# lupalab/posterior-matching

Measured on AMD Instinct MI355X. Metric: training images/sec, PM-VAE MNIST bs=256 per GPU (ELBO / PM matching-LL in `aux`), higher is better.
Workload: dtype bf16x3; 1 GPU; configs/pm_vae_mnist.py: conv PM-VAE 28x28x1, latent 32, TriL posterior, AR-GMM partial posterior, Bernoulli decoder; full train step (fwd+loss+bwd+Adam); per_gpu_batch=256, global_batch=256, parallelism=dp1, launch=launch_plan_2streams, params=2101969, rccl_ranks=1

## Files before the change

include/pmhip.h:

```cpp
#ifndef PMHIP_H
#define PMHIP_H

#ifdef __cplusplus
extern "C" {
#endif

#define PM_OK 0
#define PM_EINVAL (-1)
#define PM_ELAUNCH (-2)

#define PM_ACT_NONE 0
#define PM_ACT_LEAKY 1
#define PM_ACT_RELU 2
#define PM_ACT_GELU 3
#define PM_AUX_AFTER_RES 16

typedef void* pm_stream_t;

typedef struct pm_gather_desc {
    int B;
    int IH, IW, C;
    int OH, OW, N;
    int KH, KW;
    int a, cs, off, d;
    int wts, wcs, wns;
    int groups;
    long long in_gs, w_gs, out_gs, bias_gs;
    int in_act, out_act, aux_act;
    float slope;
    int off_x, kws;
} pm_gather_desc;

int pm_gather_gemm(pm_stream_t stream, const pm_gather_desc* d, const float* in, const float* w,
                   const float* bias, const float* aux, const float* res, float* out);

int pm_gather_wgrad(pm_stream_t stream, const pm_gather_desc* d, const float* gathered,
                    const float* dense, float* dw, float* db);

int pm_gather_gemm_bf16(pm_stream_t stream, const pm_gather_desc* d, const float* in, const void* wsplit,
                        const float* bias, const float* aux, const float* res, float* out);
int pm_gather_gemm_bf16_dual(pm_stream_t stream, const pm_gather_desc* d, const float* in, const void* wsplit,
                             const float* bias, const float* aux, const float* res, float* out, float* out2, int act2);
int pm_gemm_splitk_floats(const pm_gather_desc* d, int bf16, int in_aligned16, long long* floats);
int pm_gather_gemm_sk(pm_stream_t stream, const pm_gather_desc* d, const float* in, const float* w, const float* bias,
                      const float* aux, const float* res, float* out, float* scratch, long long scratch_floats);
int pm_gather_gemm_bf16_sk(pm_stream_t stream, const pm_gather_desc* d, const float* in, const void* wsplit,
                           const float* bias, const float* aux, const float* res, float* out, float* out2, int act2,
                           float* scratch, long long scratch_floats);
int pm_gather_gemm_bf16_insum(pm_stream_t stream, const pm_gather_desc* d, const float* in, const void* wsplit,
                              const float* bias, const float* aux, const float* res, float* out, float* in_colsum);
int pm_image_conv_insum_applies(const pm_gather_desc* d);

int pm_gather_wgrad_bf16(pm_stream_t stream, const pm_gather_desc* d, const float* gathered, const float* dense,
                         float* dw, float* db);

typedef struct pm_split_job {
    long long src_off;
    long long dst_off;
    long long plane;
    int taps, C, N, npad;
    int wts, wcs, wns;
    int first_block, num_blocks;
    int kw, kws;
    int dense_k;
} pm_split_job;
int pm_split_weights(pm_stream_t stream, const float* params, void* out_bf16, const pm_split_job* jobs_dev,
                     int njobs, int total_blocks);

int pm_thin_conv(pm_stream_t stream, const pm_gather_desc* d, const float* in, const float* w, const float* bias,
                 const float* aux, const float* res, float* out);
int pm_thin_wgrad(pm_stream_t stream, const pm_gather_desc* d, const float* gathered, const float* dense, float* dw,
                  float* db, float* db_gathered);
int pm_thin_to1_bf16(pm_stream_t stream, const pm_gather_desc* d, const float* in, const float* w, const float* bias,
                     const float* aux, const float* res, float* out);
int pm_tap_shift_add(pm_stream_t stream, const pm_gather_desc* d, const float* T, int ldt, const float* bias,
                     float* out);

int pm_gather_wgrad_table(pm_stream_t stream, const pm_gather_desc* d, const float* gathered, const float* dense, float* dw,
                          float* db, const long long* table, int all_aligned16, int use_bf16);

int pm_query_gemm_plan(const pm_gather_desc* d, int in_aligned16, int* bm, int* bn, int* vec);
int pm_query_wgrad_plan(const pm_gather_desc* d, int gathered_aligned16, int dense_aligned16, int* rc, int* rn,
                        int* vec, int* dvec, int* workgroups);

int pm_mask_concat(pm_stream_t stream, const float* x, const float* b, float* out, long long R, int C, int Cb);

int pm_tril_sample_kl_fwd(pm_stream_t stream, const float* params, const float* eps, float* z, float* kl, int B, int k);
int pm_tril_sample_kl_bwd(pm_stream_t stream, const float* params, const float* eps, const float* dz,
                          const float* g_kl, float* dparams, int B, int k);
int pm_tril_sample_kl_bwd2(pm_stream_t stream, const float* params, const float* eps, const float* dz, const float* dz2,
                           const float* g_kl, float* dparams, int B, int k);
int pm_tril_logprob_fwd(pm_stream_t stream, const float* params, const float* z, float* lp, int B, int k);
int pm_tril_logprob_bwd(pm_stream_t stream, const float* params, const float* z, const float* g,
                        float* dparams, float* dz , int B, int k);

int pm_diag_gaussian_sample_kl_fwd(pm_stream_t stream, const float* params, const float* eps, float* z, float* kl, int B, int k);
int pm_diag_gaussian_sample_kl_bwd(pm_stream_t stream, const float* params, const float* eps, const float* dz,
                                   const float* g_kl, float* dparams, int B, int k);
int pm_diag_gaussian_logprob_fwd(pm_stream_t stream, const float* params, const float* z, float* lp, int B, int k);
int pm_diag_gaussian_logprob_bwd(pm_stream_t stream, const float* params, const float* z, const float* g, float* dparams,
                                 float* dz, int B, int k);

int pm_bernoulli_ll_fwd(pm_stream_t stream, const float* logits, const float* x, float* ll, int B, int D);
int pm_bernoulli_ll_bwd(pm_stream_t stream, const float* logits, const float* x, const float* g, float* dpre,
                        int B, int D, int act, float slope);
int pm_bernoulli_ll_fwd_bwd(pm_stream_t stream, const float* logits, const float* x, const float* g, float* ll, float* dpre,
                            int B, int D, int act, float slope);

int pm_normal_ll_fwd(pm_stream_t stream, const float* loc, const float* x, const float* log_scale, float* ll, int B,
                     int D, float scale_eps);
int pm_normal_ll_bwd(pm_stream_t stream, const float* loc, const float* x, const float* log_scale, const float* g,
                     float* dloc, float* d_log_scale, int B, int D, float scale_eps);
int pm_normal_ll_bwd_det(pm_stream_t stream, const float* loc, const float* x, const float* log_scale, const float* g,
                         float* dloc, float* d_log_scale, int B, int D, float scale_eps, float* scratch);

int pm_argmm_build_input(pm_stream_t stream, const float* z, const float* ctx, float* inp, int B, int k, int ctx_dim);
int pm_argmm_input_bwd(pm_stream_t stream, const float* dinp, float* dz, float* dctx, int B, int k, int ctx_dim,
                       int accumulate_dz, const float* ctx, int ctx_act, float slope);
int pm_gmm_logprob_fwd(pm_stream_t stream, const float* head, const float* z, float* mll, int B, int k, int nc);
int pm_gmm_logprob_bwd(pm_stream_t stream, const float* head, const float* z, const float* g, float* dhead,
                       float* dz, int B, int k, int nc, int accumulate_dz);

int pm_vq_select(pm_stream_t stream, const float* z, const float* emb, const float* dots, float* e2, int* idx,
                 float* quant, float* commit_grad, float* sqerr, float* counts, float* dw, int N, int D, int K,
                 float commit_coef);
int pm_vq_dw_exact_floats(int N, int D, int K, long long* floats);
int pm_vq_dw_exact(pm_stream_t stream, const float* z, const int* idx, float* dw, int N, int D, int K, float* scratch,
                   long long scratch_floats);
int pm_embed_bwd_sorted(pm_stream_t stream, const int* idx, const float* dout, float* dtable, long long rows, int F, int K,
                        float* scratch, long long scratch_floats);
int pm_vq_ema_update(pm_stream_t stream, const float* counts, const float* dw, float* cs_hidden, float* cs_avg,
                     float* dw_hidden, float* dw_avg, float* emb, int* counter, int D, int K, float decay,
                     float epsilon);
int pm_vq_lookup(pm_stream_t stream, const int* idx, const float* emb, float* quant, int N, int D, int K);
// ... 276 lines not shown
```

posterior_matching_amd/_lib.py:

```python
from __future__ import annotations

import ctypes as C
import os

_HERE = os.path.dirname(os.path.abspath(__file__))
LIB_PATH = os.environ.get("PM_LIB_PATH") or os.path.join(_HERE, "lib", "libpmhip.so")

ACT_NONE, ACT_LEAKY, ACT_RELU, ACT_GELU = 0, 1, 2, 3
AUX_AFTER_RES = 16
LEAKY_SLOPE = 0.01


class PmHipError(RuntimeError):
    pass


class GatherDesc(C.Structure):

    _fields_ = [
        ("B", C.c_int),
        ("IH", C.c_int), ("IW", C.c_int), ("C", C.c_int),
        ("OH", C.c_int), ("OW", C.c_int), ("N", C.c_int),
        ("KH", C.c_int), ("KW", C.c_int),
        ("a", C.c_int), ("cs", C.c_int), ("off", C.c_int), ("d", C.c_int),
# ... 12 lines not shown
        ("low", C.c_float), ("high", C.c_float),
        ("period_or_steps", C.c_int), ("delay_or_begin", C.c_int),
        ("matching_coef", C.c_float),
        ("grad_scale", C.c_float),
    ]


class AdamCfg(C.Structure):
    _fields_ = [
        ("b1", C.c_float), ("b2", C.c_float), ("eps", C.c_float), ("weight_decay", C.c_float),
        ("lr_init", C.c_float), ("lr_decay_rate", C.c_float), ("lr_transition_steps", C.c_float),
        ("grad_scale", C.c_float),
        ("lr_kind", C.c_int), ("lr_end", C.c_float), ("zero_grad", C.c_int),
    ]


class MaskComponent(C.Structure):

    _fields_ = [
        ("kind", C.c_int), ("p", C.c_float),
        ("y1", C.c_int), ("x1", C.c_int), ("y2", C.c_int), ("x2", C.c_int),
        ("size", C.c_int), ("min_prop", C.c_float), ("max_prop", C.c_float), ("cum_weight", C.c_float),
    ]


class VdvaeBlockIO(C.Structure):

    _fields_ = [
        ("x", C.c_void_p), ("x2", C.c_void_p), ("res", C.c_void_p), ("xpre", C.c_void_p), ("xg_out", C.c_void_p),
        ("h", C.c_void_p * 3), ("g", C.c_void_p * 3), ("out", C.c_void_p),
        ("w", C.c_void_p * 4), ("plane", C.c_longlong * 4), ("bias", C.c_void_p * 4),
        ("Cin", C.c_int), ("Cout", C.c_int), ("Ca", C.c_int), ("dense_k3", C.c_int),
    ]


class SplitJob(C.Structure):

    _fields_ = [
        ("src_off", C.c_longlong), ("dst_off", C.c_longlong), ("plane", C.c_longlong),
        ("taps", C.c_int), ("C", C.c_int), ("N", C.c_int), ("npad", C.c_int),
        ("wts", C.c_int), ("wcs", C.c_int), ("wns", C.c_int),
        ("first_block", C.c_int), ("num_blocks", C.c_int),
        ("kw", C.c_int), ("kws", C.c_int), ("dense_k", C.c_int),
    ]


class WgradPart(C.Structure):

    _fields_ = [
        ("w", C.c_void_p), ("b", C.c_void_p), ("bg", C.c_void_p),
        ("w_stride", C.c_longlong), ("b_stride", C.c_longlong), ("bg_stride", C.c_longlong),
        ("nslots", C.c_int),
    ]


class ColsumJob(C.Structure):
    _fields_ = [("x", C.c_void_p), ("part", C.c_void_p), ("part_stride", C.c_longlong), ("M", C.c_longlong),
                ("N", C.c_int), ("nslots", C.c_int)]


class ReduceJob(C.Structure):

    _fields_ = [
        ("src", C.c_void_p), ("stride", C.c_longlong), ("g_off", C.c_longlong),
        ("count", C.c_int), ("nslots", C.c_int),
    ]


_P = C.c_void_p
_I = C.c_int
_LL = C.c_longlong
_F = C.c_float

SIGNATURES = {
    "pm_gather_gemm": [_P, C.POINTER(GatherDesc), _P, _P, _P, _P, _P, _P],
    "pm_gather_wgrad": [_P, C.POINTER(GatherDesc), _P, _P, _P, _P],
    "pm_gather_gemm_bf16": [_P, C.POINTER(GatherDesc), _P, _P, _P, _P, _P, _P],
    "pm_gather_gemm_bf16_dual": [_P, C.POINTER(GatherDesc), _P, _P, _P, _P, _P, _P, _P, _I],
    "pm_gemm_splitk_floats": [C.POINTER(GatherDesc), _I, _I, C.POINTER(C.c_longlong)],
    "pm_gather_gemm_sk": [_P, C.POINTER(GatherDesc), _P, _P, _P, _P, _P, _P, _P, C.c_longlong],
    "pm_gather_gemm_bf16_sk": [_P, C.POINTER(GatherDesc), _P, _P, _P, _P, _P, _P, _P, _I, _P, C.c_longlong],
    "pm_gather_gemm_bf16_insum": [_P, C.POINTER(GatherDesc), _P, _P, _P, _P, _P, _P, _P],
    "pm_image_conv_insum_applies": [C.POINTER(GatherDesc)],
    "pm_split_weights": [_P, _P, _P, _P, _I, _I],
    "pm_gather_wgrad_bf16": [_P, C.POINTER(GatherDesc), _P, _P, _P, _P],
    "pm_gather_wgrad_table": [_P, C.POINTER(GatherDesc), _P, _P, _P, _P, _P, _I, _I],
    "pm_wgrad_part_slots": [C.POINTER(GatherDesc), _P, _P, _I, _I, _I, C.POINTER(_I)],
    "pm_gather_wgrad_part": [_P, C.POINTER(GatherDesc), _P, _P, _P, _I, _I, C.POINTER(WgradPart)],
    "pm_thin_wgrad_part_slots": [C.POINTER(GatherDesc), _P, _P, C.POINTER(_I)],
    "pm_thin_wgrad_part": [_P, C.POINTER(GatherDesc), _P, _P, C.POINTER(WgradPart)],
    "pm_colsum_part_slots": [_LL, _I, C.POINTER(_I)],
    "pm_colsum_part": [_P, _P, _LL, _I, _P, _LL, _I],
    "pm_colsum_part_multi": [_P, _P, _I],
    "pm_reduce_partials": [_P, _P, _I, _P],
    "pm_adam_step_jobs": [_P, _P, _I, _P, _P, _P, _P, _LL, _P, C.POINTER(AdamCfg)],
    "pm_thin_conv": [_P, C.POINTER(GatherDesc), _P, _P, _P, _P, _P, _P],
    "pm_thin_wgrad": [_P, C.POINTER(GatherDesc), _P, _P, _P, _P, _P],
    "pm_thin_to1_bf16": [_P, C.POINTER(GatherDesc), _P, _P, _P, _P, _P, _P],
    "pm_tap_shift_add": [_P, C.POINTER(GatherDesc), _P, _I, _P, _P],
    "pm_mask_concat": [_P, _P, _P, _P, _LL, _I, _I],
    "pm_tril_sample_kl_fwd": [_P, _P, _P, _P, _P, _I, _I],
    "pm_tril_sample_kl_bwd": [_P, _P, _P, _P, _P, _P, _I, _I],
    "pm_tril_logprob_fwd": [_P, _P, _P, _P, _I, _I],
    "pm_tril_logprob_bwd": [_P, _P, _P, _P, _P, _P, _I, _I],
    "pm_diag_gaussian_sample_kl_fwd": [_P, _P, _P, _P, _P, _I, _I],
    "pm_diag_gaussian_sample_kl_bwd": [_P, _P, _P, _P, _P, _P, _I, _I],
    "pm_diag_gaussian_logprob_fwd": [_P, _P, _P, _P, _I, _I],
    "pm_diag_gaussian_logprob_bwd": [_P, _P, _P, _P, _P, _P, _I, _I],
    "pm_bernoulli_ll_fwd": [_P, _P, _P, _P, _I, _I],
    "pm_bernoulli_ll_bwd": [_P, _P, _P, _P, _P, _I, _I, _I, _F],
    "pm_bernoulli_ll_fwd_bwd": [_P, _P, _P, _P, _P, _P, _I, _I, _I, _F],
    "pm_tril_sample_kl_bwd2": [_P, _P, _P, _P, _P, _P, _P, _I, _I],
    "pm_normal_ll_fwd": [_P, _P, _P, _P, _P, _I, _I, _F],
    "pm_normal_ll_bwd": [_P, _P, _P, _P, _P, _P, _P, _I, _I, _F],
    "pm_normal_ll_bwd_det": [_P, _P, _P, _P, _P, _P, _P, _I, _I, _F, _P],
    "pm_vq_select": [_P, _P, _P, _P, _P, _P, _P, _P, _P, _P, _P, _I, _I, _I, _F],
    "pm_vq_dw_exact": [_P, _P, _P, _P, _I, _I, _I, _P, C.c_longlong],
    "pm_embed_bwd_sorted": [_P, _P, _P, _P, C.c_longlong, _I, _I, _P, C.c_longlong],
    "pm_vq_dw_exact_floats": [_I, _I, _I, C.POINTER(C.c_longlong)],
    "pm_vq_ema_update": [_P, _P, _P, _P, _P, _P, _P, _P, _P, _I, _I, _F, _F],
    "pm_vq_lookup": [_P, _P, _P, _P, _I, _I, _I],
    "pm_vqvae_loss": [_P, _P, _P, _P, _I, _I, _I, _I, _F, _F, _P, _P],
    "pm_argmm_build_input": [_P, _P, _P, _P, _I, _I, _I],
    "pm_argmm_input_bwd": [_P, _P, _P, _P, _I, _I, _I, _I, _P, _I, _F],
    "pm_gmm_logprob_fwd": [_P, _P, _P, _P, _I, _I, _I],
    "pm_gmm_logprob_bwd": [_P, _P, _P, _P, _P, _P, _I, _I, _I, _I],
    "pm_embed_fwd": [_P, _P, _P, _P, _LL, _I, _I],
    "pm_embed_bwd": [_P, _P, _P, _P, _LL, _I, _I],
    "pm_embed_bwd_exact": [_P, _P, _P, _P, _LL, _I, _I, _P],
    "pm_concat_elu_fwd": [_P, _P, _P, _P, _P, _LL, _I, _I],
    "pm_concat_elu_bwd": [_P, _P, _P, _P, _P, _P, _P, _LL, _I, _I, _I, _P],
    "pm_gate_bwd_rows_sum": [_P, _P, _P, _P, _P, _P, _LL, _I, _I],
    "pm_concat_elu_fwd_philox": [_P, _P, _P, _P, _LL, _I, _I, _F, C.c_ulonglong, _P, _I],
    "pm_concat_elu_bwd_philox": [_P, _P, _P, _P, _P, _P, _LL, _I, _I, _I, _P, _F, C.c_ulonglong, _P, _I],
    "pm_gate_fwd": [_P, _P, _P, _P, _P, _LL, _I, _I],
    "pm_gate_fwd_ce": [_P, _P, _P, _P, _P, _P, _LL, _I, _I],
    "pm_gate_bwd": [_P, _P, _P, _P, _P, _LL, _I, _I],
    "pm_rows_sum": [_P, _P, _P, _LL, _I, _I],
    "pm_rows_sum_multi": [_P, _P, _I, _P, C.c_longlong, _I, _I],
    "pm_groups_sum": [_P, _P, _P, _LL, _I, _LL, _I],
    "pm_elu_fwd": [_P, _P, _P, _LL],
    "pm_elu_bwd": [_P, _P, _P, _P, _LL, _I],
    "pm_categorical_ll_fwd": [_P, _P, _P, _P, _P, _LL, _I, _I],
    "pm_categorical_ll_bwd": [_P, _P, _P, _P, _P, _P, _LL, _I, _I],
    "pm_neg_mean_loss": [_P, _P, _I, _F, _P, _P],
    "pm_categorical_sample": [_P, _P, _P, _P, _LL, _I, _I, _I],
    "pm_impute_blend": [_P, _P, _P, _P, _LL, _I, _LL, _I, _I, _F, _F],
    "pm_imputation_psnr": [_P, _P, _P, _P, _LL, _I, _LL, _F],
    "pm_gumbel_fill": [_P, _P, _LL, C.c_ulonglong, _P, _I],
    "pm_mlp_pair_bf16": [_P, _P, _P, _P, _P, _P, _P, _P, _P, _P, _LL, _I, _I, _I, _I, _I, _F],
    "pm_info_gain_inputs": [_P, _P, _P, _P, _P, _I, _I, _I],
    "pm_gaussian_entropy": [_P, _P, _P, _LL, _I, _I, _I],
    "pm_info_gain_finish": [_P, _P, _P, _P, _I, _I],
    "pm_sample_project_fwd": [_P, _P, _P, _I, _P, _P, _P, _P, _P, _P, _P, _LL, _I, _I, _I],
    "pm_sample_project_bwd": [_P, _P, _P, _I, _P, _P, _P, _F, _P, _P, _LL, _I, _I],
    "pm_mlp_chain_bf16": [_P, _P, _I, _P, _P, _P, _P, _LL, _I, _I, _I, _I, _F],
    "pm_repeat_rows": [_P, _P, _P, _LL, _I, _LL],
    "pm_sigmoid": [_P, _P, _P, _LL],
    "pm_bernoulli_ll_rep_fwd": [_P, _P, _P, _P, _P, _I, _I, _I, _I],
    "pm_normal_ll_rep_fwd": [_P, _P, _P, _P, _P, _P, _I, _I, _I, _I, _F],
    "pm_std_normal_logprob": [_P, _P, _P, _LL, _I],
    "pm_logmeanexp3": [_P, _P, _P, _P, _P, _I, _I, _I],
    "pm_gmm_sample_step": [_P, _P, _P, _P, _P, _LL, _I, _I, _I],
    "pm_diag_logprob_acc": [_P, _P, _I, _P, _P, _LL, _I, _I, _F],
    "pm_segment_wsum": [_P, _P, _P, _P, _I, _I, _F, _I],
    "pm_image_mask_mixture": [_P, _P, _I, _I, _I, C.POINTER(MaskComponent), _I, C.c_ulonglong, _P, _I, _P, _P,
# ... 108 lines not shown
```

posterior_matching_amd/models/networks.py:

```python
from __future__ import annotations

from typing import Any, Dict, List, Optional, Sequence, Tuple

import torch

from .. import ops
from ..ops import ACT_LEAKY, ACT_NONE, ACT_RELU, LayerGeom
from .core import Feat, Module, ParamStore


class ConvEncoder(Module):

    def __init__(self, conv_layers: Sequence[Tuple[int, int, int]], name: Optional[str] = None):
        super().__init__(name)
        self._conv_layers = [tuple(l) for l in conv_layers]

    def build(self, store: ParamStore, prefix: str, in_shape) -> Tuple[int, ...]:
        if len(in_shape) != 3:
            raise ValueError(f"ConvEncoder expects [H, W, C] inputs, got {tuple(in_shape)}")
        self.attach(store, prefix)
        h, w, c = in_shape
        self.geoms: List[LayerGeom] = []
        self._ws = []
        n = len(self._conv_layers)
        for i, (f, k, s) in enumerate(self._conv_layers):
            g = LayerGeom.conv(h, w, c, f, k, s, "VALID" if i == n - 1 else "SAME")
            store.add(f"{prefix}/conv_{i}/w", g.weight_shape, fan_in=k * k * c)
            store.add(f"{prefix}/conv_{i}/b", (f,))
            self.geoms.append(g)
            self._ws.append((store.request_split(f"{prefix}/conv_{i}/w", g, "fwd"),
                             store.request_split(f"{prefix}/conv_{i}/w", g, "dgrad")))
            h, w, c = g.OH, g.OW, f
        return (h, w, c)

    def __call__(self, x: Feat, is_training: bool = False) -> Feat:
        assert x.in_act == ACT_NONE
        B = x.t.shape[0]
        self._x = x
        self._outs = []
        h = x.t
        for i, g in enumerate(self.geoms):
            out = self.buf(f"out_{i}", (B, g.OH, g.OW, g.CO))
            ops.layer_forward(g, h, self.P(f"conv_{i}/w"), self.P(f"conv_{i}/b"), out, out_act=ACT_LEAKY,
                              wsplit=self.store.split_view(self._ws[i][0]))
            self._outs.append(out)
            h = out
        return Feat(h, ACT_NONE, ACT_LEAKY)

    def backward(self, dpre: torch.Tensor, need_input_grad: bool = False) -> Optional[torch.Tensor]:
        B = dpre.shape[0]
        for i in reversed(range(len(self.geoms))):
            g = self.geoms[i]
            inp = self._outs[i - 1] if i > 0 else self._x.t
            lent = self.ws.wgrad_stream
            if i in getattr(self, "own_stream_wgrad", ()):
                self.ws.wgrad_stream = None
            self.wgrad(g, inp, dpre, self.G(f"conv_{i}/w"), self.G(f"conv_{i}/b"))
            self.ws.wgrad_stream = lent
            if i > 0:
                dprev = self.buf(f"dpre_{i - 1}", (B, g.IH, g.IW, g.CI))
                ops.layer_dgrad(g, dpre, self.P(f"conv_{i}/w"), dprev, aux=inp, aux_act=ACT_LEAKY,
                                wsplit=self.store.split_view(self._ws[i][1]))
                dpre = dprev
            elif need_input_grad:
                dprev = self.buf("dx", (B, g.IH, g.IW, g.CI))
                ops.layer_dgrad(g, dpre, self.P(f"conv_{i}/w"), dprev, aux=self._x.t, aux_act=self._x.grad_act,
                                wsplit=self.store.split_view(self._ws[i][1]))
                return dprev
        return None


class ConvDecoder(Module):

    def __init__(self, conv_layers: Sequence[Tuple[int, int, int]], name: Optional[str] = None):
        super().__init__(name)
        self._conv_layers = [tuple(l) for l in conv_layers]

    def build(self, store: ParamStore, prefix: str, in_shape) -> Tuple[int, ...]:
        if len(in_shape) != 1:
            raise ValueError(f"ConvDecoder expects [Z] inputs, got {tuple(in_shape)}")
        self.attach(store, prefix)
        h, w, c = 1, 1, in_shape[0]
        self.geoms = []
        self._ws = []
        for i, (f, k, s) in enumerate(self._conv_layers):
            g = LayerGeom.conv_t(h, w, c, f, k, s, "VALID" if i == 0 else "SAME")
            store.add(f"{prefix}/conv_t_{i}/w", g.weight_shape, fan_in=k * k * c)
            store.add(f"{prefix}/conv_t_{i}/b", (f,))
            self.geoms.append(g)
            self._ws.append((store.request_split(f"{prefix}/conv_t_{i}/w", g, "fwd"),
                             store.request_split(f"{prefix}/conv_t_{i}/w", g, "dgrad")))
            h, w, c = g.OH, g.OW, f
        return (h, w, c)

    def __call__(self, x: Feat, is_training: bool = False) -> Feat:
        B = x.t.shape[0]
        self._x = x
        self._outs = []
        h = x.t
        for i, g in enumerate(self.geoms):
            out = self.buf(f"out_{i}", (B, g.OH, g.OW, g.CO))
            tmp = self.buf(f"taps_{i}", (B, g.IH, g.IW, g.k * g.k)) if (g.CO == 1 and g.s == 1 and i > 0) else None
            ops.layer_forward(g, h, self.P(f"conv_t_{i}/w"), self.P(f"conv_t_{i}/b"), out,
                              in_act=x.in_act if i == 0 else ACT_NONE, out_act=ACT_LEAKY,
                              wsplit=self.store.split_view(self._ws[i][0]), tmp=tmp)
            self._outs.append(out)
            h = out
        return Feat(h, ACT_NONE, ACT_LEAKY)

    def backward(self, dpre: torch.Tensor, need_input_grad: bool = True, lend=None) -> Optional[torch.Tensor]:
        B = dpre.shape[0]
        ops.colsum_defer_begin()
        try:
            return self._backward(dpre, need_input_grad, lend, B)
        finally:
            ops.colsum_defer_flush()

    def _backward(self, dpre, need_input_grad, lend, B):
        for i in reversed(range(len(self.geoms))):
            g = self.geoms[i]
            inp = self._outs[i - 1] if i > 0 else self._x.t
            if lend is not None and i < lend[1]:
                self.ws.wgrad_stream = lend[0]
            wsd = self.store.split_view(self._ws[i][1])
# ... 297 lines not shown
```

posterior_matching_amd/ops.py:

```python
from __future__ import annotations

import ctypes as C
import os
import math
from dataclasses import dataclass
from typing import Optional

import torch

from . import _lib
from ._lib import ACT_GELU, ACT_LEAKY, ACT_NONE, ACT_RELU, AUX_AFTER_RES, LEAKY_SLOPE, GatherDesc


def _stream() -> int:
    return torch.cuda.current_stream().cuda_stream


def _ptr(t: Optional[torch.Tensor]):
    if t is None:
        return None
    assert t.is_cuda and t.dtype == torch.float32 and t.is_contiguous(), "expects contiguous f32 device tensors"
    return t.data_ptr()


# ... 551 lines not shown
    tag = work = None
    if _timer is not None:
        v = [C.c_int() for _ in range(5)]
        lib.pm_query_wgrad_plan(C.byref(desc), int(gathered.data_ptr() % 16 == 0),
                                int(dense.data_ptr() % 16 == 0), *[C.byref(x) for x in v])
        tag = f"gather_wgrad_kernel<{v[0].value},{v[1].value},{_MODES[v[2].value]},{v[3].value}>"
        work = {"flops": _algorithmic_flops(desc), "bytes": _nbytes(gathered, dense, dw), "detail": _detail(desc)}
    ns = C.c_int()
    part = None
    if lib.pm_wgrad_part_slots(C.byref(desc), _ptr(gathered), _ptr(dense), 0, al, 0, C.byref(ns)) == 0:
        part = _part_arenas(desc, dw, db, ns.value)
    if part is not None:
        _call("pm_gather_wgrad_part", C.byref(desc), _ptr(gathered), _ptr(dense), None, al, 0, C.byref(part), tag=tag, work=work)
        _part_done(part)
        return
    _call("pm_gather_wgrad", C.byref(desc), _ptr(gathered), _ptr(dense), _ptr(dw), _ptr(db), tag=tag, work=work)


def _lane_form(d: GatherDesc) -> bool:
    return (d.groups == 1 and d.d == 1 and d.a == 1 and d.KH == d.KW and d.KH in (3, 5) and d.C in (1, 2)
            and d.N <= 32 and d.OW <= 128 and d.OH <= 128 and d.off_x == d.off and d.kws == d.KW)


def _to1_form(d: GatherDesc) -> bool:
    return (d.groups == 1 and d.d == 1 and d.a == 1 and d.N == 1 and d.C % 4 == 0 and d.OW <= 256
            and d.off_x == d.off and d.kws == d.KW
            and (d.KH * d.KW * d.C + d.KH * (d.OW + d.KW - 1) * (d.C + 4)) * 4 <= 64 * 1024)


def _thin_ok(d: GatherDesc) -> bool:
    if _lane_form(d) or _to1_form(d):
        return True
    return (d.groups == 1 and d.d == 1 and d.KH * d.KW * d.C <= 64 and d.N <= 32 and d.N % 8 == 0
            and d.off_x == d.off and d.kws == d.KW)


def thin_conv(desc: GatherDesc, inp, w, bias, aux, res, out) -> None:
    tag = work = None
    if _timer is not None:
        tag = ("thin_to1_kernel" if _to1_form(desc) and inp.data_ptr() % 16 == 0 else
               f"thin_conv_lane_kernel<{desc.C}, {desc.KH}>" if _lane_form(desc) else "thin_conv_kernel")
        work = {"flops": _algorithmic_flops(desc), "bytes": _nbytes(inp, aux, res, out), "detail": _detail(desc)}
    _call("pm_thin_conv", C.byref(desc), _ptr(inp), _ptr(w), _ptr(bias), _ptr(aux), _ptr(res), _ptr(out), tag=tag,
          work=work)


def layer_forward(g: LayerGeom, x, w, b, out, in_act=ACT_NONE, out_act=ACT_NONE, res=None, wsplit=None,
                  tmp=None, out2=None, act2=ACT_NONE, **group_kw) -> None:
    B = group_kw.pop("B", None) or x.shape[0]
    d = g._desc(B, "fwd", **group_kw)
    d.in_act, d.out_act = in_act, out_act
    if (wsplit is not None and _to1_form(d) and d.C in (32, 64) and d.KH * d.KW <= 32 and x.data_ptr() % 16 == 0
            and d.KH * d.IW * ((d.KH * d.KW) | 1) * 4 <= 64 * 1024):
        work = {"flops": _algorithmic_flops(d), "bytes": _nbytes(x, res, out), "detail": _detail(d)}
        _call("pm_thin_to1_bf16", C.byref(d), _ptr(x), _ptr(w), _ptr(b), None, _ptr(res), _ptr(out),
              tag=f"thin_to1_bf16_kernel<{d.C // 32}>", work=work)
        if out2 is not None:
            gelu_fwd(out, None, out2)
        return
    if _thin_ok(d):
        thin_conv(d, x, w, b, None, res, out)
        if out2 is not None:
            gelu_fwd(out, None, out2)
        return
    if g.kind == "convT" and g.CO == 1 and g.s == 1 and tmp is not None and res is None and in_act == ACT_NONE:
        taps = g.k * g.k
        dt = LayerGeom.dense(g.CI, taps)._desc(B * g.IH * g.IW, "fwd")
        dt.wts, dt.wcs, dt.wns = 0, 1, g.CI
        gather_gemm(dt, x, w, None, None, None, tmp)
        work = {"bytes": _nbytes(tmp, out), "detail": _detail(d)}
        _call("pm_tap_shift_add", C.byref(d), _ptr(tmp), taps, _ptr(b), _ptr(out), work=work)
        return
    if wsplit is not None and bf16_supported(d):
        if d.groups > 1:
            d.w_gs = wsplit.numel() // d.groups
        gather_gemm_bf16(d, x, wsplit, b, None, res, out, out2=out2, act2=act2)
    else:
        gather_gemm(d, x, w, b, None, res, out)
        if out2 is not None:
            assert act2 == ACT_GELU, "the unfused second store only exists for gelu"
            gelu_fwd(out, None, out2)


def dgrad_insum_ok(g: LayerGeom, B: int, wsplit, force: bool = False) -> bool:
    if wsplit is None or not (force or os.environ.get("PM_DGRAD_INSUM")):
        return False
    d = g._desc(B, "dgrad")
    if _thin_ok(d) or not bf16_supported(d):
        return False
    return bool(_lib.load().pm_image_conv_insum_applies(C.byref(d)))


def layer_dgrad(g: LayerGeom, dy, w, dx, aux=None, aux_act=ACT_NONE, res=None, wsplit=None, in_colsum=None, **group_kw) -> None:
    B = group_kw.pop("B", None) or dy.shape[0]
    d = g._desc(B, "dgrad", **group_kw)
    d.aux_act = aux_act if aux is not None else ACT_NONE
    aux = aux if aux_act != ACT_NONE else None
    if in_colsum is not None:
        gather_gemm_bf16(d, dy, wsplit, None, aux, res, dx, in_colsum=in_colsum)
        return
    if _thin_ok(d):
        thin_conv(d, dy, w, None, aux, res, dx)
        return
    if wsplit is not None and bf16_supported(d):
        if d.groups > 1:
            d.w_gs = wsplit.numel() // d.groups
        gather_gemm_bf16(d, dy, wsplit, None, aux, res, dx)
    else:
        gather_gemm(d, dy, w, None, aux, res, dx)


def layer_wgrad(g: LayerGeom, x, dy, dw, db, in_act=ACT_NONE, bf16: bool = True, **group_kw) -> None:
    B = group_kw.pop("B", None) or x.shape[0]
    d = g._desc(B, "wgrad", **group_kw)
    d.in_act = in_act
    if g.kind != "convT":
        gather_wgrad(d, x, dy, dw, db, bf16=bf16)
        return
    if in_act != ACT_NONE:
        raise NotImplementedError("transposed-conv weight gradient with a pending input activation")
    d = g._desc(B, "dgrad", **group_kw)
    fused = gather_wgrad(d, dy, x, dw, None, bf16=bf16, db_gathered=db)
    if db is not None and not fused:
        colsum(dy, db)


class WgradBatch:

    def __init__(self):
        self.items = {}
        self._tables = {}
        self._ptables = {}
        self.reducer = None

    def add(self, g: LayerGeom, x, dy, dw, db, bf16: bool, in_act: int = ACT_NONE) -> None:
        if g.kind == "convT":
            raise NotImplementedError("deferred weight gradients of transposed convolutions")
        B = x.shape[0]
        d = g._desc(B, "wgrad")
        use_bf16 = bool(bf16 and USE_BF16_WGRAD and _bf16_wgrad_channels(d.C) and d.N % 4 == 0 and d.d in (1, 2))
        key = (B, g.kind, g.IH, g.IW, g.CI, g.OH, g.OW, g.CO, g.KH, g.KW, g.s, g.pad, g.pad_x, g.full_kh, g.full_kw, in_act,
               use_bf16, db is not None)
        self.items.setdefault(key, []).append((g, x, dy, dw, db))

    @staticmethod
    def eligible(g: LayerGeom, d: GatherDesc) -> bool:
        return g.kind != "convT" and not _lane_form(d)

    def flush(self) -> None:
        for key, lst in self.items.items():
            g0, x0, dy0, dw0, db0 = lst[0]
            ptrs = tuple(t.data_ptr() for it in lst for t in it[1:] if t is not None)
            cached = self._tables.get((key, ptrs))
            if cached is None:
                rows = []
                for _, x, dy, dw, db in lst:
                    rows += [(x.data_ptr() - x0.data_ptr()) // 4, (dy.data_ptr() - dy0.data_ptr()) // 4,
                             (dw.data_ptr() - dw0.data_ptr()) // 4,
                             ((db.data_ptr() - db0.data_ptr()) // 4) if db is not None else 0]
                aligned = all(x.data_ptr() % 16 == 0 and dy.data_ptr() % 16 == 0 for _, x, dy, _, _ in lst)
                cached = (torch.tensor(rows, dtype=torch.int64, device=x0.device), int(aligned))
                self._tables[(key, ptrs)] = cached
            table, aligned = cached
            d = g0._desc(key[0], "wgrad", groups=len(lst))
            d.in_act = key[-3]
            tag = work = None
# ... 905 lines not shown
```

Measured before the change: 198,900 images/sec.

## Fuse first four encoder conv layers into one LDS-resident stack kernel

Adds a HIP kernel that runs the first four encoder convolutions for one image per workgroup. Intermediate activations stay in LDS as bf16 hi/lo split planes, and the later layers are computed with MFMA. This removes three or four separate conv launches plus the global-memory round trips for the intermediate inputs. Each layer's fp32 output is still written out for backward. It is gated on specific geometry, tile counts and batch size of at least 128, and needs a large dynamic LDS allocation, which limits the kernel to one block per CU.

```diff
diff --git a/include/pmhip.h b/include/pmhip.h
--- a/include/pmhip.h
+++ b/include/pmhip.h
@@ -50,6 +50,10 @@
 int pm_gather_gemm_bf16_insum(pm_stream_t stream, const pm_gather_desc* d, const float* in, const void* wsplit,
                               const float* bias, const float* aux, const float* res, float* out, float* in_colsum);
 int pm_image_conv_insum_applies(const pm_gather_desc* d);
+
+int pm_conv_stack_plan(const pm_gather_desc* layers, int nlayers, long long* lds_bytes);
+int pm_conv_stack_fwd_bf16(pm_stream_t stream, const pm_gather_desc* layers, int nlayers, const float* in, const float* w0,
+                           const void* const* wsplit, const float* const* bias, float* const* out);
 
 int pm_gather_wgrad_bf16(pm_stream_t stream, const pm_gather_desc* d, const float* gathered, const float* dense,
                          float* dw, float* db);
diff --git a/posterior_matching_amd/_lib.py b/posterior_matching_amd/_lib.py
--- a/posterior_matching_amd/_lib.py
+++ b/posterior_matching_amd/_lib.py
@@ -118,6 +118,8 @@
     "pm_gather_gemm_bf16_sk": [_P, C.POINTER(GatherDesc), _P, _P, _P, _P, _P, _P, _P, _I, _P, C.c_longlong],
     "pm_gather_gemm_bf16_insum": [_P, C.POINTER(GatherDesc), _P, _P, _P, _P, _P, _P, _P],
     "pm_image_conv_insum_applies": [C.POINTER(GatherDesc)],
+    "pm_conv_stack_plan": [C.POINTER(GatherDesc), _I, C.POINTER(C.c_longlong)],
+    "pm_conv_stack_fwd_bf16": [_P, C.POINTER(GatherDesc), _I, _P, _P, _P, _P, _P],
     "pm_split_weights": [_P, _P, _P, _P, _I, _I],
     "pm_gather_wgrad_bf16": [_P, C.POINTER(GatherDesc), _P, _P, _P, _P],
     "pm_gather_wgrad_table": [_P, C.POINTER(GatherDesc), _P, _P, _P, _P, _P, _I, _I],
diff --git a/posterior_matching_amd/csrc/pm_conv_stack.hip b/posterior_matching_amd/csrc/pm_conv_stack.hip
--- /dev/null
+++ b/posterior_matching_amd/csrc/pm_conv_stack.hip
@@ -0,0 +1,411 @@
+#include <cstdint>
+#include <cstdlib>
+#include <type_traits>
+#include "pm_common.h"
+
+namespace {
+
+constexpr int BK = 32;
+constexpr int NW = 8;
+constexpr int ROW_INVALID = -(1 << 28);
+constexpr size_t LDS_MAX = 160 * 1024;
+
+typedef __bf16 bf16x8 __attribute__((ext_vector_type(8)));
+typedef __bf16 bf16x2 __attribute__((ext_vector_type(2)));
+typedef float f32x2 __attribute__((ext_vector_type(2)));
+typedef unsigned u32x2 __attribute__((ext_vector_type(2)));
+
+__device__ __forceinline__ void split2(float a0, float a1, unsigned& hi, unsigned& lo) {
+    const unsigned h = __builtin_bit_cast(unsigned, __builtin_convertvector(f32x2{a0, a1}, bf16x2));
+    const float f0 = __builtin_bit_cast(float, h << 16);
+    const float f1 = __builtin_bit_cast(float, h & 0xffff0000u);
+    hi = h;
+    lo = __builtin_bit_cast(unsigned, __builtin_convertvector(f32x2{a0 - f0, a1 - f1}, bf16x2));
+}
+
+struct StackConv {
+    int IH, IW, C, OH, OW, N, KH, KW, a, cs, off, offx;
+    int npad, nct, wct;
+    long long plane;
+    const __bf16* ws;
+    const float* bias;
+    float* out;
+    int in_off, out_off;
+};
+
+struct StackArgs {
+    int IH, IW, OH, OW, N, off;
+    int wts, wcs, wns;
+    float slope;
+    const float* in;
+    const float* w;
+    const float* bias;
+    float* out;
+    int out_off, patch_off;
+    StackConv L[3];
+};
+
+__device__ __forceinline__ void zero_slots(char* lds, int off, int npos, int PS, int tid) {
+    if (tid < 32) {
+        __bf16* h = reinterpret_cast<__bf16*>(lds + off);
+        reinterpret_cast<unsigned*>(h + (size_t)npos * PS)[tid] = 0u;
+        reinterpret_cast<unsigned*>(h + 2 * (size_t)npos * PS + 64)[tid] = 0u;
+    }
+}
+
+template <int C0, int KS>
+__device__ __forceinline__ void lane_layer(const StackArgs& p, char* lds, int b, int tid) {
+    constexpr int NSLOT = 64 * NW / 32;
+    const int n = tid & 31, slot = tid >> 5;
+    const int PH = p.OH + KS - 1;
+    const int QX = (p.OW + 3) >> 2;
+    const int PW = 4 * QX + 4;
+    float* P = reinterpret_cast<float*>(lds + p.patch_off);
+    const float* img = p.in + (size_t)b * p.IH * p.IW * C0;
+    for (int e = tid; e < C0 * PH * PW; e += 64 * NW) {
+        const int c = e / (PH * PW);
+        const int r = e - c * PH * PW;
+        const int py = r / PW, px = r - py * PW;
+        const int gy = p.off + py, gx = p.off + px;
+        float v = 0.f;
+        if ((unsigned)gy < (unsigned)p.IH && (unsigned)gx < (unsigned)p.IW) v = img[(gy * p.IW + gx) * C0 + c];
+        P[e] = v;
+    }
+    float wr[C0][KS][KS];
+#pragma unroll
+    for (int c = 0; c < C0; ++c)
+#pragma unroll
+        for (int jy = 0; jy < KS; ++jy)
+#pragma unroll
+            for (int jx = 0; jx < KS; ++jx) wr[c][jy][jx] = p.w[(jy * KS + jx) * p.wts + c * p.wcs + n * p.wns];
+    const float bv = p.bias ? p.bias[n] : 0.f;
+    const int PS = p.N + 8;
+    unsigned short* Qh = reinterpret_cast<unsigned short*>(lds + p.out_off);
+    unsigned short* Ql = Qh + (size_t)p.OH * p.OW * PS + 64;
+    __syncthreads();
+    for (int item = slot; item < p.OH * QX; item += NSLOT) {
+        const int y = item / QX, qx = item - y * QX;
+        float acc[4] = {0.f, 0.f, 0.f, 0.f};
+#pragma unroll
+        for (int c = 0; c < C0; ++c)
+#pragma unroll
+            for (int jy = 0; jy < KS; ++jy) {
+                const float* row = P + (c * PH + y + jy) * PW + 4 * qx;
+                const f32x4 x0 = *reinterpret_cast<const f32x4*>(row);
+                const f32x4 x1 = *reinterpret_cast<const f32x4*>(row + 4);
+                const float xv[8] = {x0[0], x0[1], x0[2], x0[3], x1[0], x1[1], x1[2], x1[3]};
+#pragma unroll
+                for (int jx = 0; jx < KS; ++jx)
+#pragma unroll
+                    for (int j = 0; j < 4; ++j) acc[j] = fmaf(xv[j + jx], wr[c][jy][jx], acc[j]);
+            }
+        float v[4];
+#pragma unroll
+        for (int j = 0; j < 4; ++j) {
+            float xx = acc[j] + bv;
+            xx = pm_act(xx, PM_ACT_LEAKY, p.slope);
+            asm volatile("" : "+v"(xx));
+            v[j] = xx;
+        }
+        const int nv = p.OW - 4 * qx < 4 ? p.OW - 4 * qx : 4;
+        const int pos0 = y * p.OW + 4 * qx;
+        const size_t o0 = ((size_t)b * p.OH * p.OW + pos0) * p.N + n;
+        unsigned h01, l01, h23, l23;
+        split2(v[0], v[1], h01, l01);
+        split2(v[2], v[3], h23, l23);
+        const unsigned hv[4] = {h01 & 0xffffu, h01 >> 16, h23 & 0xffffu, h23 >> 16};
+        const unsigned lv[4] = {l01 & 0xffffu, l01 >> 16, l23 & 0xffffu, l23 >> 16};
+#pragma unroll
+        for (int j = 0; j < 4; ++j)
+            if (j < nv) {
+                p.out[o0 + (size_t)j * p.N] = v[j];
+                Qh[(pos0 + j) * PS + n] = (unsigned short)hv[j];
+                Ql[(pos0 + j) * PS + n] = (unsigned short)lv[j];
+            }
+    }
+}
+
+template <int T>
+__device__ __forceinline__ void image_layer(const StackConv& L, char* lds, int b, int wave, int lane, float slope) {
+    constexpr int NSET = 4;
+    const int i = lane & 31;
+    const int h = lane >> 5;
+    const int PS = L.C + 8;
+    const int cch = L.C / BK;
+    const int nsteps = L.KH * L.KW * cch;
+    const int npos = L.IH * L.IW;
+    const __bf16* Ph = reinterpret_cast<const __bf16*>(lds + L.in_off);
+    const __bf16* Pl = Ph + (size_t)npos * PS + 64;
+    const int zoff = npos * PS;
+    const int ct = wave / L.wct, rt0 = wave - ct * L.wct;
+    const int Mi = L.OH * L.OW;
+    if (ct >= L.nct || rt0 * 32 >= Mi) return;
+    const int n = ct * 32 + i;
+    const int ncl = (n < L.npad ? n : 0) * BK + 8 * h;
+
+    bf16x8 bq[NSET][4];
+    auto load_b = [&](int s, bf16x8 (&bb)[4]) {
+        const int sc = s < nsteps ? s : nsteps - 1;
+        const __bf16* src = L.ws + (size_t)sc * L.npad * BK + ncl;
+        bb[0] = *reinterpret_cast<const bf16x8*>(src);
+        bb[1] = *reinterpret_cast<const bf16x8*>(src + L.plane);
+        bb[2] = *reinterpret_cast<const bf16x8*>(src + 16);
+        bb[3] = *reinterpret_cast<const bf16x8*>(src + L.plane + 16);
+    };
+    load_b(0, bq[0]);
+    load_b(1, bq[1]);
+    load_b(2, bq[2]);
+    load_b(3, bq[3]);
+
+    int py[T], px[T];
+#pragma unroll
+    for (int j = 0; j < T; ++j) {
+        const int m = 32 * (rt0 + j * L.wct) + i;
+        const int oy = m / L.OW, ox = m - oy * L.OW;
+        py[j] = m < Mi ? oy * L.a + L.off : ROW_INVALID;
+        px[j] = ox * L.a + L.offx;
+    }
+    f32x16 acc[T];
+#pragma unroll
+    for (int j = 0; j < T; ++j)
+#pragma unroll
+        for (int e = 0; e < 16; ++e) acc[j][e] = 0.f;
+
+    bf16x8 a[4][4];
+    struct Tap { int dy, dx, c0; };
+    int wky = 0, wkx = 0, wcc = 0;
+    auto advance = [&]() -> Tap {
+        const Tap t{wky * L.cs, wkx * L.cs, wcc * BK};
+        if (++wcc == cch) {
+            wcc = 0;
+            if (++wkx == L.KW) {
+                wkx = 0;
+                ++wky;
+            }
+        }
+        return t;
+    };
+    auto read_a = [&](const Tap& k, int j, bf16x8 (&aa)[4]) {
+        const int iy = py[j] + k.dy, ix = px[j] + k.dx;
+        const bool ok = (unsigned)iy < (unsigned)L.IH && (unsigned)ix < (unsigned)L.IW;
+        const int o = (ok ? (iy * L.IW + ix) * PS + k.c0 : zoff) + 8 * h;
+        aa[0] = *reinterpret_cast<const bf16x8*>(Ph + o);
+        aa[1] = *reinterpret_cast<const bf16x8*>(Ph + o + 16);
+        aa[2] = *reinterpret_cast<const bf16x8*>(Pl + o);
+        aa[3] = *reinterpret_cast<const bf16x8*>(Pl + o + 16);
+    };
+    Tap t0, t1, t2;
+    auto step = [&](int s, auto uc) {
+        constexpr int u = decltype(uc)::value;
+#pragma unroll
+        for (int j = 0; j < T; ++j) {
+            const int cur = (u * T + j) & 3;
+            const int jn = j + 2;
+            read_a(jn / T == 0 ? t0 : jn / T == 1 ? t1 : t2, jn % T, a[(cur + 2) & 3]);
+            acc[j] = __builtin_amdgcn_mfma_f32_32x32x16_bf16(bq[u][0], a[cur][0], acc[j], 0, 0, 0);
+            acc[j] = __builtin_amdgcn_mfma_f32_32x32x16_bf16(bq[u][1], a[cur][0], acc[j], 0, 0, 0);
+            acc[j] = __builtin_amdgcn_mfma_f32_32x32x16_bf16(bq[u][0], a[cur][2], acc[j], 0, 0, 0);
+            acc[j] = __builtin_amdgcn_mfma_f32_32x32x16_bf16(bq[u][2], a[cur][1], acc[j], 0, 0, 0);
+            acc[j] = __builtin_amdgcn_mfma_f32_32x32x16_bf16(bq[u][3], a[cur][1], acc[j], 0, 0, 0);
+            acc[j] = __builtin_amdgcn_mfma_f32_32x32x16_bf16(bq[u][2], a[cur][3], acc[j], 0, 0, 0);
+        }
+        t0 = t1;
+        t1 = t2;
+        t2 = advance();
+        load_b(s + NSET, bq[u]);
+        __builtin_amdgcn_sched_barrier(0);
+    };
+    using U0 = std::integral_constant<int, 0>;
+    using U1 = std::integral_constant<int, 1>;
+    using U2 = std::integral_constant<int, 2>;
+    using U3 = std::integral_constant<int, 3>;
+    static_assert(T == 1 || T == 2 || T == 4, "item index mod 4 must be static inside a group of NSET k-steps");
+    t0 = advance();
+    t1 = advance();
+    t2 = advance();
+    read_a(t0, 0, a[0]);
+    read_a(T == 1 ? t1 : t0, T == 1 ? 0 : 1, a[1]);
+    int s0 = 0;
+    for (; s0 + NSET <= nsteps; s0 += NSET) {
+        step(s0, U0{});
+        step(s0 + 1, U1{});
+        step(s0 + 2, U2{});
+        step(s0 + 3, U3{});
+    }
+    if (s0 < nsteps) {
+        step(s0, U0{});
+        if (s0 + 1 < nsteps) {
+            step(s0 + 1, U1{});
+            if (s0 + 2 < nsteps) step(s0 + 2, U2{});
+        }
+    }
+
+    const int PSq = L.N + 8;
+    __bf16* Qh = reinterpret_cast<__bf16*>(lds + (L.out_off >= 0 ? L.out_off : 0));
+    __bf16* Ql = Qh + (size_t)Mi * PSq + 64;
+#pragma unroll
+    for (int j = 0; j < T; ++j) {
+        const int m = 32 * (rt0 + j * L.wct) + i;
+        f32x4 v[4];
+#pragma unroll
+        for (int g = 0; g < 4; ++g) {
+            const int c = ct * 32 + 8 * g + 4 * h;
+            const int cc = c < L.N ? c : 0;
+            const f32x4 bv = L.bias ? *reinterpret_cast<const f32x4*>(L.bias + cc) : f32x4{0.f, 0.f, 0.f, 0.f};
+#pragma unroll
+            for (int q = 0; q < 4; ++q) {
+                float x = acc[j][4 * g + q] + bv[q];
+                x = pm_act(x, PM_ACT_LEAKY, slope);
+                asm volatile("" : "+v"(x));
+                v[g][q] = x;
+            }
+        }
+        if (m >= Mi) continue;
+        float* orow = L.out + ((long long)b * Mi + m) * L.N;
+#pragma unroll
+        for (int g = 0; g < 4; ++g) {
+            const int c = ct * 32 + 8 * g + 4 * h;
+            if (c >= L.N) continue;
+            *reinterpret_cast<f32x4*>(orow + c) = v[g];
+            if (L.out_off >= 0) {
+                unsigned h0, l0, h1, l1;
+                split2(v[g][0], v[g][1], h0, l0);
+                split2(v[g][2], v[g][3], h1, l1);
+                *reinterpret_cast<u32x2*>(Qh + m * PSq + c) = u32x2{h0, h1};
+                *reinterpret_cast<u32x2*>(Ql + m * PSq + c) = u32x2{l0, l1};
+            }
+        }
+    }
+}
+
+template <int C0, int KS, int T2, int T3, int T4>
+__global__ __launch_bounds__(64 * NW, 1) void conv_stack_fwd_bf16_kernel(StackArgs p) {
+    extern __shared__ __attribute__((aligned(16))) float dsm[];
+    char* lds = reinterpret_cast<char*>(dsm);
+    const int tid = threadIdx.x;
+    const int lane = tid & 63, wave = tid >> 6;
+    const int b = blockIdx.x;
+    zero_slots(lds, p.out_off, p.OH * p.OW, p.N + 8, tid);
+    lane_layer<C0, KS>(p, lds, b, tid);
+    __syncthreads();
+    zero_slots(lds, p.L[0].out_off, p.L[0].OH * p.L[0].OW, p.L[0].N + 8, tid);
+    image_layer<T2>(p.L[0], lds, b, wave, lane, p.slope);
+    __syncthreads();
+    zero_slots(lds, p.L[1].out_off, p.L[1].OH * p.L[1].OW, p.L[1].N + 8, tid);
+    image_layer<T3>(p.L[1], lds, b, wave, lane, p.slope);
+    __syncthreads();
+    image_layer<T4>(p.L[2], lds, b, wave, lane, p.slope);
+}
+
+struct StackPlan {
+    size_t lds;
+    int c0, t[3];
+};
+
+inline size_t planes_bytes(int npos, int C) { return 2 * ((size_t)npos * (C + 8) + 64) * 2; }
+inline size_t align16(size_t x) { return (x + 15) & ~(size_t)15; }
+
+bool plan_stack(const pm_gather_desc* d, int nl, StackPlan& sp, StackArgs* args) {
+    if (!d || nl != 4) return false;
+    const int B = d[0].B;
+    if (B < 1) return false;
+    for (int l = 0; l < 4; ++l) {
+        const pm_gather_desc& x = d[l];
+        if (x.B != B || x.groups != 1 || x.d != 1 || x.cs != 1 || x.off_x != x.off || x.kws != x.KW) return false;
+        if (x.in_act != PM_ACT_NONE || x.out_act != PM_ACT_LEAKY || x.aux_act != PM_ACT_NONE || x.slope != d[0].slope)
+            return false;
+        if (x.a < 1 || x.IH < 1 || x.IW < 1 || x.OH < 1 || x.OW < 1 || x.C < 1 || x.N < 1 || x.KH < 1 || x.KW < 1) return false;
+        if (x.wts < 0 || x.wcs < 0 || x.wns < 0) return false;
+        if ((long long)B * x.OH * x.OW * x.N >= 0x7fffffffLL || (long long)B * x.IH * x.IW * x.C >= 0x7fffffffLL) return false;
+        if (l > 0 && (x.IH != d[l - 1].OH || x.IW != d[l - 1].OW || x.C != d[l - 1].N)) return false;
+        if (x.off < -64 || x.off > 64) return false;
+    }
+    const pm_gather_desc& f = d[0];
+    if (f.a != 1 || f.KH != 5 || f.KW != 5 || (f.C != 1 && f.C != 2) || f.N != 32 || f.OW > 128 || f.OH > 128) return false;
+    if ((long long)(f.KH * f.KW - 1) * f.wts + (long long)(f.C - 1) * f.wcs + 31LL * f.wns >= 0x7fffffffLL) return false;
+    size_t in_bytes[3];
+    for (int l = 1; l < 4; ++l) {
+        const pm_gather_desc& x = d[l];
+        if (x.C % BK != 0 || x.KH * x.KW < 4 || x.KH > 16 || x.KW > 16 || x.IH < x.KH || x.IW < x.KW || x.OH * x.OW < 32)
+            return false;
+        if (x.N % 4 != 0) return false;
+        if (x.KH * x.KW * (x.C / BK) > 2048) return false;
+        const int nct = (x.N + 31) / 32;
+        if (nct > NW || NW % nct != 0) return false;
+        const int wct = NW / nct;
+        const int rt = (x.OH * x.OW + 31) / 32;
+        int t = (rt + wct - 1) / wct;
+        if (t == 3) t = 4;
+        if (t > 4) return false;
+        sp.t[l - 1] = t;
+        in_bytes[l - 1] = planes_bytes(x.IH * x.IW, x.C);
+        if (args) {
+            StackConv& L = args->L[l - 1];
+            L.IH = x.IH; L.IW = x.IW; L.C = x.C; L.OH = x.OH; L.OW = x.OW; L.N = x.N; L.KH = x.KH; L.KW = x.KW;
+            L.a = x.a; L.cs = x.cs; L.off = x.off; L.offx = x.off_x;
+            L.npad = nct * 32; L.nct = nct; L.wct = wct;
+            L.plane = (long long)x.KH * x.KW * (x.C / BK) * BK * L.npad;
+        }
+    }
+    if (sp.t[0] != 1 || sp.t[1] != 2 || sp.t[2] != 1) return false;
+    const size_t patch = (size_t)f.C * (f.OH + f.KH - 1) * (4 * ((f.OW + 3) / 4) + 4) * 4;
+    const size_t x_bytes = align16(in_bytes[0] > in_bytes[2] ? in_bytes[0] : in_bytes[2]);
+    const size_t y_bytes = in_bytes[1] > patch ? in_bytes[1] : patch;
+    sp.lds = x_bytes + y_bytes;
+    if (sp.lds > LDS_MAX) return false;
+    sp.c0 = f.C;
+    if (args) {
+        args->IH = f.IH; args->IW = f.IW; args->OH = f.OH; args->OW = f.OW; args->N = f.N; args->off = f.off;
+        args->wts = f.wts; args->wcs = f.wcs; args->wns = f.wns; args->slope = f.slope;
+        args->out_off = 0;
+        args->patch_off = (int)x_bytes;
+        args->L[0].in_off = 0;                 args->L[0].out_off = (int)x_bytes;
+        args->L[1].in_off = (int)x_bytes;      args->L[1].out_off = 0;
+        args->L[2].in_off = 0;                 args->L[2].out_off = -1;
+    }
+    return true;
+}
+
+inline bool al16(const void* p) { return (reinterpret_cast<uintptr_t>(p) & 15) == 0; }
+
+template <int C0>
+void launch_stack(hipStream_t s, const StackPlan& sp, const StackArgs& a, int B) {
+    static bool attr = false;
+    if (!attr) {
+        (void)hipFuncSetAttribute(reinterpret_cast<const void*>(&conv_stack_fwd_bf16_kernel<C0, 5, 1, 2, 1>),
+                                  hipFuncAttributeMaxDynamicSharedMemorySize, (int)LDS_MAX);
+        attr = true;
+    }
+    PM_KTAG("conv_stack_fwd_bf16_kernel<%d, 5, 1, 2, 1>", C0);
+    hipLaunchKernelGGL((conv_stack_fwd_bf16_kernel<C0, 5, 1, 2, 1>), dim3((unsigned)B), dim3(64 * NW), sp.lds, s, a);
+}
+
+}
+
+extern "C" int pm_conv_stack_plan(const pm_gather_desc* layers, int nlayers, long long* lds_bytes) {
+    StackPlan sp;
+    if (!plan_stack(layers, nlayers, sp, nullptr)) return PM_EINVAL;
+    if (lds_bytes) *lds_bytes = (long long)sp.lds;
+    return PM_OK;
+}
+
+extern "C" int pm_conv_stack_fwd_bf16(pm_stream_t stream, const pm_gather_desc* layers, int nlayers, const float* in,
+                                      const float* w0, const void* const* wsplit, const float* const* bias, float* const* out) {
+    StackPlan sp;
+    StackArgs a;
+    if (!plan_stack(layers, nlayers, sp, &a) || !in || !w0 || !wsplit || !bias || !out) return PM_EINVAL;
+    for (int l = 0; l < 4; ++l) {
+        if (!out[l] || !al16(out[l]) || (bias[l] && !al16(bias[l]))) return PM_EINVAL;
+        if (l > 0 && (!wsplit[l] || !al16(wsplit[l]))) return PM_EINVAL;
+    }
+    a.in = in; a.w = w0; a.bias = bias[0]; a.out = out[0];
+    for (int l = 1; l < 4; ++l) {
+        a.L[l - 1].ws = reinterpret_cast<const __bf16*>(wsplit[l]);
+        a.L[l - 1].bias = bias[l];
+        a.L[l - 1].out = out[l];
+    }
+    hipStream_t s = (hipStream_t)stream;
+    if (sp.c0 == 1) launch_stack<1>(s, sp, a, layers[0].B);
+    else launch_stack<2>(s, sp, a, layers[0].B);
+    return pm_check_launch("pm_conv_stack_fwd_bf16");
+}
diff --git a/posterior_matching_amd/models/networks.py b/posterior_matching_amd/models/networks.py
--- a/posterior_matching_amd/models/networks.py
+++ b/posterior_matching_amd/models/networks.py
@@ -39,7 +39,18 @@
         self._x = x
         self._outs = []
         h = x.t
-        for i, g in enumerate(self.geoms):
+        first = 0
+        ws = [self.store.split_view(self._ws[i][0]) for i in range(min(4, len(self.geoms)))]
+        biases = [self.P(f"conv_{i}/b") for i in range(len(ws))]
+        if (len(ws) == 4 and all(w is not None for w in ws[1:]) and all(b.data_ptr() % 16 == 0 for b in biases)
+                and ops.conv_stack_applies(self.geoms[:4], B)):
+            outs = [self.buf(f"out_{i}", (B, g.OH, g.OW, g.CO)) for i, g in enumerate(self.geoms[:4])]
+            ops.conv_stack_fwd(self.geoms[:4], h, self.P("conv_0/w"), biases[0], ws[1:], biases[1:], outs)
+            self._outs.extend(outs)
+            h = outs[3]
+            first = 4
+        for i in range(first, len(self.geoms)):
+            g = self.geoms[i]
             out = self.buf(f"out_{i}", (B, g.OH, g.OW, g.CO))
             ops.layer_forward(g, h, self.P(f"conv_{i}/w"), self.P(f"conv_{i}/b"), out, out_act=ACT_LEAKY,
                               wsplit=self.store.split_view(self._ws[i][0]))
diff --git a/posterior_matching_amd/ops.py b/posterior_matching_amd/ops.py
--- a/posterior_matching_amd/ops.py
+++ b/posterior_matching_amd/ops.py
@@ -657,6 +657,46 @@
             gelu_fwd(out, None, out2)
 
 
+def _conv_stack_descs(geoms, B: int):
+    descs = (GatherDesc * 4)()
+    for i, g in enumerate(geoms):
+        d = g._desc(B, "fwd")
+        d.in_act, d.out_act = ACT_NONE, ACT_LEAKY
+        descs[i] = d
+    return descs
+
+
+def conv_stack_lds(geoms, B: int) -> Optional[int]:
+    if len(geoms) != 4:
+        return None
+    n = C.c_longlong(0)
+    if _lib.load().pm_conv_stack_plan(_conv_stack_descs(geoms, B), 4, C.byref(n)) != 0:
+        return None
+    return n.value
+
+
+def conv_stack_applies(geoms, B: int) -> bool:
+    if os.environ.get("PM_NO_CONV_STACK") or B < 128:
+        return False
+    return conv_stack_lds(geoms, B) is not None
+
+
+def conv_stack_fwd(geoms, x, w0, b0, wsplits, biases, outs) -> None:
+    B = x.shape[0]
+    descs = _conv_stack_descs(geoms, B)
+    for t in outs:
+        _ptr(t)
+    ws = (C.c_void_p * 4)(None, *[w.data_ptr() for w in wsplits])
+    bs = (C.c_void_p * 4)(*[_ptr(b) for b in [b0] + list(biases)])
+    os_ = (C.c_void_p * 4)(*[_ptr(t) for t in outs])
+    work = None
+    if _timer is not None:
+        work = {"flops": sum(_algorithmic_flops(d) for d in descs), "bytes": _nbytes(x, *outs),
+                "detail": " | ".join(_detail(d) for d in descs)}
+    _call("pm_conv_stack_fwd_bf16", descs, 4, _ptr(x), _ptr(w0), ws, bs, os_,
+          tag=f"conv_stack_fwd_bf16_kernel<{geoms[0].CI}, 5, 1, 2, 1>", work=work)
+
+
 def dgrad_insum_ok(g: LayerGeom, B: int, wsplit, force: bool = False) -> bool:
     if wsplit is None or not (force or os.environ.get("PM_DGRAD_INSUM")):
         return False
```

Result: faster. 203,700 images/sec, median of 6 (+2.4%).
